# E3SM-Project/PAM

Hardware: AMD Instinct MI355X
Metric: cell-updates/sec (AWFL dycore step) (higher is better)
Workload: dtype f64; 1 GPU; AWFL supercell idealized, nens=1024/GPU, 32x32x60 L60, NT=1, fp64; scaling=weak, nens_total=1024, nens_per_gpu=1024, nx=32, ny=32, nz=60, num_tracers=1, parallelism=nens-shard x1, ranks_seen=1, limiter_input=0, fct_rows_flagged_last_stage=0, fct_rows=983040, lanes=member+xsweep

## Files before the change

### pam_amd/csrc/awfl_device.h

```cpp
#pragma once
#include <math.h>
#include <stdint.h>
#include <string.h>
#include <type_traits>
#include "awfl_constants.h"

#if defined(__HIPCC__)
#define PAMA_D __device__ __forceinline__
#else
#define PAMA_D inline
#endif

namespace pama {

constexpr int HS = 3;
constexpr int MAXT = 50;
constexpr int FLUX_THREADS = 256;
constexpr int FLUX_WAVES = FLUX_THREADS / 64;
#ifndef PAMA_FLUX_NF
#define PAMA_FLUX_NF 2
#endif
constexpr int FLUX_NF = PAMA_FLUX_NF;
constexpr int FLUX_MAX_SPAN = 64;
constexpr int VZ_STRIDE = 31;
// ... 1448 lines not shown
    for (int n = 0; n < NF; n++) T.nq[n] = uni(q[n] + on)[eu];
    T.ruf = uni(ruf_line + (long long)(c == nx ? 0 : c) * P.sx)[eu];
    const int cc = c > c0 ? c - 1 : c0;
    const long long o = pbase + (long long)cc * P.sx, ix = fbase + (long long)cc * P.sx;
    T.rho_in = 0.0; T.rho_0 = 0.0; T.rho_new = 1.0;
    if (PHASE == 2) {
      T.rho_in = uni(pr + o)[eu];
      T.rho_0 = (STAGE > 1) ? uni(r0 + o)[eu] : 0.0;
      T.rho_new = uni(rn + o)[eu];
    }
#pragma unroll
    for (int n = 0; n < NF; n++) {
      T.yl[n] = have_y ? uni(fyt[n] + ix)[eu] : 0.0;
      T.yh[n] = have_y ? uni(fyt[n] + ix + jp1)[eu] : 0.0;
      T.zl[n] = uni(fzt[n] + ix)[eu];
      T.zh[n] = uni(fzt[n] + ix + P.sz)[eu];
      T.sd[n] = (PHASE == 1) ? uni(seed + (long long)tt[n] * P.ncell + ix)[eu] : 0.0;
      T.q_0[n] = (PHASE == 2 && STAGE > 1) ? uni(q0p[n] + o)[eu] : 0.0;
      T.m_jm1[n] = T.m_jp1[n] = T.m_km1[n] = T.m_kp1[n] = T.m_new[n] = 1.0;
      if (PHASE == 2) {
        T.m_new[n] = uni(mline[n] + (long long)(c == nx ? 0 : c) * P.sx)[eu];
        if (have_y) { T.m_jm1[n] = uni(mline[n] + (long long)cc * P.sx + jm1)[eu]; T.m_jp1[n] = uni(mline[n] + (long long)cc * P.sx + jp1)[eu]; }
        if (zlo) T.m_km1[n] = uni(mline[n] + (long long)cc * P.sx - P.sz)[eu];
        if (zhi) T.m_kp1[n] = uni(mline[n] + (long long)cc * P.sx + P.sz)[eu];
      }
    }
  };
  Trip Tn;
  if (AHEAD) load_trip(c0, Tn);
#pragma clang loop unroll(disable)
  for (int c = c0; c <= c1; c++) {
    Trip T;
    if (AHEAD) {
      T = Tn;
      if (c < c1) load_trip(c + 1, Tn);
    } else {
      load_trip(c, T);
    }
    double L[NF], R[NF];
    double ruf = T.ruf;
    if (have_close && c == c1) ruf = ruf_close;
    const int cc = c > c0 ? c - 1 : c0;
    const long long ix = fbase + (long long)cc * P.sx;
    const double rho_in = T.rho_in, rho_0 = T.rho_0, rho_new = T.rho_new;
    const double (&nq)[NF] = T.nq, (&yl)[NF] = T.yl, (&yh)[NF] = T.yh, (&zl)[NF] = T.zl, (&zh)[NF] = T.zh, (&sd)[NF] = T.sd, (&q_0)[NF] = T.q_0;
    const double (&m_new)[NF] = T.m_new, (&m_jm1)[NF] = T.m_jm1, (&m_jp1)[NF] = T.m_jp1, (&m_km1)[NF] = T.m_km1, (&m_kp1)[NF] = T.m_kp1;
#pragma unroll
    for (int n = 0; n < NF; n++) weno5_const(w[n], wc, L[n], R[n]);
    const bool up = ruf > 0.0;
    const double rrho = (PHASE == 2) ? fast_rcp(rho_new) : 0.0;
#pragma unroll
    for (int n = 0; n < NF; n++) {
      const double F = mul_rn(ruf, up ? prevR[n] : L[n]);
      if (c > c0) {
        if (PHASE == 1) {
          own_multiplier_cell<true>(P, tt[n], mult, rows, k, j, cc, e, eu, ix, F_prev[n], F, yl[n], yh[n], zl[n], zh[n], sd[n], dzk, rdzk, dt_stage);
        } else {
          const double f_x = limited_flux(F_prev[n], mA[n], mB[n], cc == 0);
          const double f_xp1 = limited_flux(F, mB[n], m_new[n], cc == nx - 1);
          double f_y = 0.0, f_yp1 = 0.0;
          if (have_y) {
            f_y = limited_flux(yl[n], m_jm1[n], mB[n], j == 0);
            f_yp1 = limited_flux(yh[n], mB[n], m_jp1[n], j == P.ny - 1);
          }
          const double f_z = limited_flux(zl[n], m_km1[n], mB[n], false);
          const double f_zp1 = limited_flux(zh[n], mB[n], m_kp1[n], false);
          double v, new_seed;
          tracer_new_value<STAGE>(P, tt[n], f_x, f_xp1, f_y, f_yp1, f_z, f_zp1, w[n][1], q_0[n], rho_in, rho_0, rdzk, dt_dyn, v, new_seed);
          uniw(seed + (long long)tt[n] * P.ncell + ix)[eu] = new_seed;
          store_adv_u(P, prim_out, P_TR0 + tt[n], k, cu0 + (long long)cc * P.sx, eu, v * rrho, v * rrho);
        }
      }
      F_prev[n] = F;
      prevR[n] = R[n];
      mA[n] = mB[n];
      mB[n] = m_new[n];
#pragma unroll
      for (int s = 0; s < 4; s++) w[n][s] = w[n][s + 1];
      w[n][4] = nq[n];
    }
  }
}

template <int STAGE, bool FOLD = false>
PAMA_D void flux_x_update_body(const Params &P, const double *__restrict__ prim_in, const double *__restrict__ prim0,
                               double *__restrict__ prim_out, double *__restrict__ fx, const double *__restrict__ fy,
                               const double *__restrict__ fz, double *__restrict__ seed, double *__restrict__ mult,
                               const FctRows &rows, int line, int e, int c0, int span, double dt_dyn, double dt_stage,
                               bool tracers_inline) {
  const unsigned eu = member_offset(e);
  const WenoConsts wc = weno_consts();
  const int nx = P.nx;
  const int c1 = (c0 + span < nx) ? c0 + span : nx;
  const int k = uni_int(line / P.ny), j = line - k * P.ny;
  const long long cu0 = (long long)j * P.sy;
  const long long pbase = (long long)(k + HS) * P.sz + cu0;
  const long long fbase = (long long)k * P.sz + cu0;
  const long long jp1 = (j == P.ny - 1) ? -(long long)(P.ny - 1) * P.sy : P.sy;
  const long long ke = (long long)k * P.nens + e;
  const double dzk = P.dz[ke];
  const double rdzk = fast_rcp(dzk);
  const double gcoef = gravity_coef(P, ke);
  const bool have_y = !P.sim2d;
  double ruf_close = 0.0;
  double *ruf_line = fx + fbase;
  auto cell_off = [&](int c) -> long long { return pbase + (long long)(c < 0 ? c + nx : (c >= nx ? c - nx : c)) * P.sx; };

  {
    constexpr int NQ = 4;
    const double *pr = prim_in + (long long)P_RHO * P.prim_fs;
    const double *pp = prim_in + (long long)P_PRES * P.prim_fs;
    const double *r0 = prim0 + (long long)P_RHO * P.prim_fs;
    double *out_rho = prim_out + (long long)P_RHO * P.prim_fs, *out_rt = prim_out + (long long)P_PRES * P.prim_fs;
    double wm[5], wp[5], wq[NQ][5], wt[5];
    const int tr = P.idWV;
    const double *pt = prim_in + (long long)(P_TR0 + tr) * P.prim_fs;
    double *flt = fx + (long long)(5 + tr) * P.ncell + fbase;
    const bool more_tracers = P.nt > 1;
    auto load_cell = [&](long long o, double &m, double &p, double (&qv)[NQ]) {
#pragma unroll
      for (int n = 0; n < NQ; n++) qv[n] = uni(prim_in + (long long)(P_U + n) * P.prim_fs + o)[eu];
      m = mul_rn(uni(pr + o)[eu], qv[0]);
      p = uni(pp + o)[eu];
    };
#pragma unroll
    for (int s = 0; s < 5; s++) {
      double qv[NQ];
      load_cell(cell_off(c0 - 3 + s), wm[s], wp[s], qv);
#pragma unroll
      for (int n = 0; n < NQ; n++) wq[n][s] = qv[n];
      wt[s] = uni(pt + cell_off(c0 - 3 + s))[eu];
    }
    double prevR_m, prevR_p, prevR_q[NQ], prevR_t;
    {
      double L;
      weno5_const(wm, wc, L, prevR_m);
      weno5_const(wp, wc, L, prevR_p);
      weno5_const(wt, wc, L, prevR_t);
#pragma unroll
      for (int n = 0; n < NQ; n++) {
        if (n == 1 && !have_y) { prevR_q[n] = 0.0; continue; }
        weno5_const(wq[n], wc, L, prevR_q[n]);
      }
      double nm, np_, nq[NQ];
      load_cell(cell_off(c0 + 2), nm, np_, nq);
      const double nt0 = uni(pt + cell_off(c0 + 2))[eu];
#pragma unroll
      for (int s = 0; s < 4; s++) {
        wm[s] = wm[s + 1]; wp[s] = wp[s + 1]; wt[s] = wt[s + 1];
#pragma unroll
        for (int n = 0; n < NQ; n++) wq[n][s] = wq[n][s + 1];
      }
      wm[4] = nm; wp[4] = np_; wt[4] = nt0;
#pragma unroll
      for (int n = 0; n < NQ; n++) wq[n][4] = nq[n];
    }
    double F_prev[1 + NQ], Ft_prev = 0.0;
#pragma unroll
    for (int l = 0; l <= NQ; l++) F_prev[l] = 0.0;
    struct CellIn { double rho_in, rho_0, q0[NQ], y0l, y0h, z0l, z0h, dy[1 + NQ], dz[1 + NQ], tyl, tyh, tzl, tzh, tseed, tq0; };
    const double *fyt = fy + (long long)(5 + tr) * P.ncell, *fzt = fz + (long long)(5 + tr) * P.fz_fs;
    const double *pt0 = prim0 + (long long)(P_TR0 + tr) * P.prim_fs;
    const double *sdt = seed + (long long)tr * P.ncell;
    auto load_in = [&](int cc, CellIn &ci) {
      const long long o = pbase + (long long)cc * P.sx, ix = fbase + (long long)cc * P.sx;
      ci.rho_in = uni(pr + o)[eu];
      ci.rho_0 = (STAGE > 1) ? uni(r0 + o)[eu] : 0.0;
#pragma unroll
      for (int n = 0; n < NQ; n++) ci.q0[n] = (STAGE > 1) ? uni(prim0 + (long long)(P_U + n) * P.prim_fs + o)[eu] : 0.0;
      ci.y0l = have_y ? uni(fy + ix)[eu] : 0.0;
      ci.y0h = have_y ? uni(fy + ix + jp1)[eu] : 0.0;
      ci.z0l = uni(fz + ix)[eu];
      ci.z0h = uni(fz + ix + P.sz)[eu];
#pragma unroll
      for (int l = 1; l <= NQ; l++) {
        ci.dy[l] = (have_y && !FOLD) ? uni(fy + (long long)l * P.ncell + ix)[eu] : 0.0;
        ci.dz[l] = (l == 2 && !have_y) ? 0.0 : uni(fz + (long long)l * P.fz_fs + ix)[eu];
      }
      ci.tyl = have_y ? uni(fyt + ix)[eu] : 0.0;
      ci.tyh = have_y ? uni(fyt + ix + jp1)[eu] : 0.0;
      ci.tzl = uni(fzt + ix)[eu];
      ci.tzh = uni(fzt + ix + P.sz)[eu];
      ci.tseed = uni(sdt + ix)[eu];
      ci.tq0 = (STAGE > 1) ? uni(pt0 + o)[eu] : 0.0;
    };
    auto finish = [&](int cc, const CellIn &ci, const double (&Flo)[1 + NQ], const double (&Fhi)[1 + NQ], double m_in_u,
                      double v_in, double w_in, double th_in, double Ft_lo, double Ft_hi, double qt_in) {
      const long long o = pbase + (long long)cc * P.sx;
      const double q0 = rk_combine<STAGE>(ci.rho_0, ci.rho_in, dt_dyn,
                                          flux_divergence(P, Flo[0], Fhi[0], ci.y0l, ci.y0h, ci.z0l, ci.z0h, rdzk));
      const double rrho = fast_rcp(q0);
      uniw(out_rho + o)[eu] = q0;
      const double q_in[NQ] = {0.0, v_in, w_in, th_in};
#pragma unroll
      for (int n = 0; n < NQ; n++) {
        const int l = 1 + n;
        double tend = FOLD ? flux_divergence_g(P, Flo[l], Fhi[l], ci.dz[l]) : flux_divergence_d(P, Flo[l], Fhi[l], ci.dy[l], ci.dz[l], rdzk);
        if (l == 3) tend = add_gravity(P, tend, ci.rho_in, gcoef);
        if (l == 2 && P.sim2d) tend = 0.0;
        const double m_in = (n == 0) ? m_in_u : mul_rn(q_in[n], ci.rho_in);
        const double m_0 = (STAGE > 1) ? mul_rn(ci.q0[n], ci.rho_0) : 0.0;
        const double v = rk_combine<STAGE>(m_0, m_in, dt_dyn, tend);
        store_adv_u(P, prim_out, P_U + n, k, cu0 + (long long)cc * P.sx, eu, v * rrho, (l == 3) ? 0.0 : v * rrho);
        if (l == 4) uniw(out_rt + o)[eu] = v;
      }
      finish_tracer_cell<STAGE>(P, tr, prim_out, seed, mult, rows, k, j, cc, e, eu, cu0 + (long long)cc * P.sx, fbase + (long long)cc * P.sx,
                                Ft_lo, Ft_hi, ci.tyl, ci.tyh, ci.tzl, ci.tzh, ci.tseed, qt_in, ci.tq0, ci.rho_in, ci.rho_0, rrho, dzk,
                                rdzk, dt_dyn, dt_stage);
    };
#pragma clang loop unroll(disable)
    for (int c = c0; c <= c1; c++) {
      double nm, np_, nq[NQ];
      load_cell(cell_off(c + 3), nm, np_, nq);
      const double nt0 = uni(pt + cell_off(c + 3))[eu];
      CellIn ci;
      load_in(c > c0 ? c - 1 : c0, ci);
      double Lm, Rm, Lp, Rp, Lq[NQ], Rq[NQ];
      weno5_const(wm, wc, Lm, Rm);
      weno5_const(wp, wc, Lp, Rp);
#pragma unroll
      for (int n = 0; n < NQ; n++) {
        if (n == 1 && !have_y) { Lq[n] = Rq[n] = 0.0; continue; }
        weno5_const(wq[n], wc, Lq[n], Rq[n]);
      }
      double Lt, Rt;
      weno5_const(wt, wc, Lt, Rt);
      double ruf, ppf, F[1 + NQ];
      acoustic_face(prevR_m, Lm, prevR_p, Lp, false, ruf, ppf);
      const bool up = ruf > 0.0;
      const double Ft = mul_rn(ruf, up ? prevR_t : Lt);
      if (c < c1) {
        if (more_tracers) uniw(ruf_line + (long long)c * P.sx)[eu] = ruf;
        uniw(flt + (long long)c * P.sx)[eu] = Ft;
      }
      ruf_close = ruf;
      F[0] = ruf;
      F[1] = fma(ruf, up ? prevR_q[0] : Lq[0], ppf);
#pragma unroll
      for (int n = 1; n < NQ; n++) F[1 + n] = mul_rn(ruf, up ? prevR_q[n] : Lq[n]);
      if (c > c0) finish(c - 1, ci, F_prev, F, wm[1], wq[1][1], wq[2][1], wq[3][1], Ft_prev, Ft, wt[1]);
#pragma unroll
      for (int l = 0; l <= NQ; l++) F_prev[l] = F[l];
      Ft_prev = Ft;
      prevR_m = Rm; prevR_p = Rp; prevR_t = Rt;
#pragma unroll
      for (int n = 0; n < NQ; n++) prevR_q[n] = Rq[n];
#pragma unroll
      for (int s = 0; s < 4; s++) {
        wm[s] = wm[s + 1]; wp[s] = wp[s + 1]; wt[s] = wt[s + 1];
#pragma unroll
        for (int n = 0; n < NQ; n++) wq[n][s] = wq[n][s + 1];
      }
      wm[4] = nm; wp[4] = np_; wt[4] = nt0;
#pragma unroll
      for (int n = 0; n < NQ; n++) wq[n][4] = nq[n];
    }
  }

  if (tracers_inline) {
    for (int i = 0; i < P.nt - 1; i += FLUX_NF) {
      const int fa[2] = {4 + further_tracer(P, i), 4 + further_tracer(P, i + 1)};
      if (i + 1 < P.nt - 1) x_tracer_sweep<2, STAGE, 1>(P, prim_in, prim0, prim_out, fx, fy, fz, seed, mult, rows, line, e, c0, span, fa, dt_dyn, dt_stage, true, ruf_close);
      else x_tracer_sweep<1, STAGE, 1>(P, prim_in, prim0, prim_out, fx, fy, fz, seed, mult, rows, line, e, c0, span, fa, dt_dyn, dt_stage, true, ruf_close);
    }
  }
}

struct XTileGeom {
  int W;
  int nmb;
  int tc;
  int halo;
  int ntl;
  int lpb;
};
PAMA_HD int xtile_rows(const XTileGeom &G) { return G.tc + 2 * G.halo; }
PAMA_HD int xtile_threads(const XTileGeom &G) { return G.W * xtile_rows(G) * G.lpb; }
PAMA_HD XTileGeom xtile_geometry(const Params &P, int w_req, int tc_req, int lpb_req, int ncu = 0) {
  XTileGeom G;
  G.W = (P.nens <= 64) ? P.nens : 64;
  if (P.nens < 64 && (long long)P.nx * P.nens > 512) {
    const int nmb = (int)(((long long)P.nx * P.nens + 511) / 512), w = (P.nens + nmb - 1) / nmb;
    if (w >= 16 && P.nx * w <= 1024) G.W = w;
    else if ((long long)P.nx * P.nens > 1024) {
      const int nmb2 = (int)(((long long)P.nx * P.nens + 1023) / 1024), w2 = (P.nens + nmb2 - 1) / nmb2;
      if (w2 >= 16 && P.nx * w2 <= 1024) G.W = w2;
    }
  }
  if (w_req > 0) G.W = w_req < P.nens ? w_req : P.nens;
  if (G.W > 1024 / 3) G.W = 64;
  G.nmb = (P.nens + G.W - 1) / G.W;
  const int max_threads = 1024;
  if (tc_req <= 0 && P.nx * G.W <= max_threads) {
    G.halo = 0; G.tc = P.nx; G.ntl = 1;
    const int row = P.nx * G.W, most = max_threads / row;
    auto used = [&](int l) { return (double)(l * row) / (double)(((l * row + 63) / 64) * 64); };
    double best = 0.0;
    for (int l = 1; l <= most; l++) best = used(l) > best ? used(l) : best;
    G.lpb = most;
    for (int l = 1; l <= most; l++)
      if (used(l) >= best - 0.03 && (l * row >= 192 || l == most)) { G.lpb = l; break; }
    if (ncu > 0) {
      const long long nlines = (long long)P.nz * P.ny;
      long long best_cost = -1;
      int best_dist = 0;
      for (int l = 1; l <= most; l++) {
        if (used(l) < best - 0.03) continue;
        const int T = ((l * row + 63) / 64) * 64;
        const long long nwg = (long long)G.nmb * ((nlines + l - 1) / l);
        const long long cost = ((nwg + ncu - 1) / ncu) * T;
        const int dist = T > 256 ? T - 256 : 256 - T;
        if (best_cost < 0 || cost < best_cost || (cost == best_cost && dist < best_dist)) { best_cost = cost; best_dist = dist; G.lpb = l; }
      }
    }
    if (lpb_req > 0) G.lpb = lpb_req < most ? lpb_req : most;
    if (G.lpb < 1) G.lpb = 1;
  } else {
    G.halo = 1; G.lpb = 1;
    int tc = tc_req > 0 ? tc_req : 14;
    if (tc > P.nx) tc = P.nx;
    while (tc > 1 && (tc + 2) * G.W > max_threads) tc--;
    G.ntl = (P.nx + tc - 1) / tc;
    G.tc = tc_req > 0 ? tc : (P.nx + G.ntl - 1) / G.ntl;
  }
  return G;
}
PAMA_HD bool xtile_supported(const Params &P) { return P.prim_fs < (1ll << 28) && P.fz_fs < (1ll << 28) && (long long)P.nz * P.ny < (1ll << 30); }

struct XLane {
  int k, j, i, e;
  bool poly, face, upd;
  int slot, slot_l, slot_r;
  unsigned po, io, ke;
  int s5[5];
  int nstage;
  unsigned stage_po[3];
  int stage_el[3];
};
// ... 732 lines not shown
```

### pam_amd/csrc/awfl_kernels.hip

```cpp
#include <hip/hip_runtime.h>

#include <cmath>
#include <cstdio>
#include <cstring>
#include <atomic>
#include <map>
#include <mutex>
#include <string>
#include <vector>

#include "../../include/pam_amd_awfl.h"
#include "awfl_device.h"
#include "awfl_vertical.h"

using namespace pama;

struct EnsRange { int e0, ne; };
__device__ __forceinline__ long long to_global(long long t, int nens, EnsRange R) {
  const long long r = t / R.ne;
  return r * nens + R.e0 + (t - r * R.ne);
}

__device__ __forceinline__ bool flat_cell(const Params &P, int nlev, CellId &c) {
  const unsigned t = blockIdx.x * blockDim.x + threadIdx.x;
// ... 82 lines not shown
  double *buf;
  const double *vz;
  long long nens;
  int eb, emax;
  int tid, lane, last;
  double r[(VZ_STRIDE * 64 + 64 * ZPE_WAVES - 1) / (64 * ZPE_WAVES)];
  static constexpr int NR = (VZ_STRIDE * 64 + 64 * ZPE_WAVES - 1) / (64 * ZPE_WAVES);
  __device__ __forceinline__ double rdz(const Params &P, int k, int e) const { return P.rdz[(long long)k * P.nens + e]; }
  __device__ __forceinline__ void load(int level) {
    const double *src = vz + (long long)level * VZ_STRIDE * nens;
#pragma unroll
    for (int i = 0; i < NR; i++) {
      const int idx = tid + i * 64 * ZPE_WAVES;
      const int m = idx >> 6, l = idx & 63, em = (eb + l < emax) ? eb + l : emax;
      r[i] = (idx < VZ_STRIDE * 64) ? src[(long long)m * nens + em] : 0.0;
    }
  }
  __device__ __forceinline__ void store(int level) {
    double *dst = buf + (level & 1) * (VZ_STRIDE * 64);
#pragma unroll
    for (int i = 0; i < NR; i++) {
      const int idx = tid + i * 64 * ZPE_WAVES;
      if (idx < VZ_STRIDE * 64) dst[idx] = r[i];
    }
  }
  __device__ __forceinline__ void pass_begin(int first, int last_) {
    last = last_;
    load(first);
    store(first);
    __syncthreads();
  }
  __device__ __forceinline__ void trip_begin(int level) { if (level < last) load(level + 1); }
  __device__ __forceinline__ void trip_end(int level) {
    if (level < last) store(level + 1);
    __syncthreads();
  }
  __device__ __forceinline__ void weno(const double u[5], int level, const WenoConsts &wc, double &L, double &R) const {
    weno5_table(u, buf + (level & 1) * (VZ_STRIDE * 64) + lane, 64, wc, L, R);
  }
};
template <bool DIFF, bool FOLD>
__global__ void __launch_bounds__(64 * ZPE_WAVES, 2) awfl_fluxz_pe_kernel(Params P, EnsRange R, int spz, int nsz, int part, int npz,
                                                                              const double *__restrict__ prim, const double *__restrict__ fy,
                                                                              double *__restrict__ fz) {
  __shared__ double ztab[2 * VZ_STRIDE * 64];
  const int lane = threadIdx.x & 63;
  const int wave = __builtin_amdgcn_readfirstlane((int)(threadIdx.x >> 6));
  const int ncol = P.ny * P.nx, ncg = (ncol + ZPE_WAVES - 1) / ZPE_WAVES;
  const int per_blk = ncg * nsz * (part == 1 ? npz : 1);
  const int b = (int)blockIdx.x;
  const int blk = uni_int(b / per_blk), r1 = b - blk * per_blk;
  const int r2 = uni_int(r1 / ncg), cg = r1 - r2 * ncg;
  const int pp = uni_int(r2 / nsz), sp = r2 - pp * nsz;
  const int psel = (part == 1) ? 1 + pp : part;
  int line = cg * ZPE_WAVES + wave;
  if (line > ncol - 1) line = ncol - 1;
  const int emax = R.e0 + R.ne - 1;
  int e = R.e0 + blk * 64 + lane;
  if (e > emax) e = emax;
  ZTabLds zt;
  zt.buf = ztab; zt.vz = P.vz; zt.nens = P.nens; zt.eb = R.e0 + blk * 64; zt.emax = emax;
  zt.tid = (int)threadIdx.x; zt.lane = lane; zt.last = 0;
  flux_line_body_zt<2, DIFF, ZTabLds, FOLD>(P, prim, fz, member_lane<2>(P, line, e), sp * spz, spz, psel, zt, fy);
}

__global__ void __launch_bounds__(256) awfl_fct_kernel(Params P, EnsRange R, const double *__restrict__ fx,
                                                       const double *__restrict__ fy, const double *__restrict__ fz,
                                                       const double *__restrict__ seed, double *__restrict__ mult,
                                                       FctRows rows, double dt, int t0) {
  fct_rows_resolve(rows);
  CellId c;
  if (grid_cell(P, R, c)) fct_mult_body(P, fx, fy, fz, seed, mult, rows, dt, c, t0);
}
template <int STAGE>
__global__ void __launch_bounds__(256) awfl_update_kernel(Params P, EnsRange R, const double *prim_in,
                                                          const double *prim0, double *prim_out,
                                                          const double *__restrict__ fx, const double *__restrict__ fy,
                                                          const double *__restrict__ fz, const double *__restrict__ mult,
                                                          FctRows rows, double *__restrict__ seed, double dt_dyn) {
  fct_rows_resolve(rows);
  CellId c;
  if (grid_cell(P, R, c)) update_body<STAGE>(P, prim_in, prim0, prim_out, fx, fy, fz, mult, rows, seed, dt_dyn, c);
}
template <int STAGE, bool FOLD>
__global__ void __launch_bounds__(FLUX_THREADS, 2) awfl_xupd_kernel(Params P, EnsRange R, const double *__restrict__ prim_in,
                                                                     const double *__restrict__ prim0,
                                                                     double *__restrict__ prim_out, double *__restrict__ fx,
                                                                     const double *__restrict__ fy,
                                                                     const double *__restrict__ fz, double *__restrict__ seed,
                                                                     double *__restrict__ mult, FctRows rows, double dt_dyn,
                                                                     double dt_stage, int tracers_inline, int span, int nspan) {
  fct_rows_resolve(rows);
  const int u = __builtin_amdgcn_readfirstlane((int)(blockIdx.x * FLUX_WAVES + (threadIdx.x >> 6)));
  const SweepUnits U = sweep_units(P.nz, P.ny, R.ne, nspan, 1);
  const SweepUnits::Unit w = U.decode(u, false);
  const int sp = U.span(w);
  const SweepUnits::Lane m = U.place(w.grp);
  const int el = m.blk * 64 + (int)(threadIdx.x & 63);
  if (U.holds(m, el))
    flux_x_update_body<STAGE, FOLD>(P, prim_in, prim0, prim_out, fx, fy, fz, seed, mult, rows, m.line, R.e0 + el, sp * span, span,
                                    dt_dyn, dt_stage, tracers_inline != 0);
}
template <int STAGE, int PHASE, int G, bool AHEAD = false>
__device__ __forceinline__ void xtr_block(const Params &P, EnsRange R, const double *__restrict__ prim_in,
                                          const double *__restrict__ prim0, double *__restrict__ prim_out,
                                          const double *__restrict__ fx, const double *__restrict__ fy,
                                          const double *__restrict__ fz, double *__restrict__ seed,
                                          double *__restrict__ mult, const FctRows &rows, double dt_dyn,
                                          double dt_stage, int ngroups, int span, int nspan, int block) {
  static_assert(G == 1 || G == 2 || G == 4, "one, two or four tracers per wavefront");
  static_assert(!AHEAD || G == 2, "the one-trip-ahead form exists for pairs only");
  const int u = __builtin_amdgcn_readfirstlane((int)(block * FLUX_WAVES + (threadIdx.x >> 6)));
  const SweepUnits U = sweep_units(P.nz, P.ny, R.ne, nspan, ngroups);
  const SweepUnits::Unit w = U.decode(u);
  const int sp = U.span(w);
  const SweepUnits::Lane m = U.place(w.grp);
  const int el = m.blk * 64 + (int)(threadIdx.x & 63);
  if (!U.holds(m, el)) return;
  if constexpr (G == 2) {
    const int fa[2] = {4 + further_tracer(P, 2 * w.sel), 4 + further_tracer(P, 2 * w.sel + 1)};
    if (2 * w.sel + 1 < P.nt - 1)
      x_tracer_sweep<2, STAGE, PHASE, AHEAD>(P, prim_in, prim0, prim_out, fx, fy, fz, seed, mult, rows, m.line, R.e0 + el, sp * span, span, fa, dt_dyn, dt_stage, false, 0.0);
    else
      x_tracer_sweep<1, STAGE, PHASE, AHEAD>(P, prim_in, prim0, prim_out, fx, fy, fz, seed, mult, rows, m.line, R.e0 + el, sp * span, span, fa, dt_dyn, dt_stage, false, 0.0);
  } else {
    const int first = G * w.sel, left = P.nt - 1 - first;
    const int fa[4] = {4 + further_tracer(P, first), 4 + further_tracer(P, first + 1), 4 + further_tracer(P, first + 2), 4 + further_tracer(P, first + 3)};
    if (G == 4 && left >= 4)
      x_tracer_sweep<4, STAGE, PHASE, AHEAD>(P, prim_in, prim0, prim_out, fx, fy, fz, seed, mult, rows, m.line, R.e0 + el, sp * span, span, fa, dt_dyn, dt_stage, false, 0.0);
    else if (G == 4 && left == 3)
      x_tracer_sweep<3, STAGE, PHASE, AHEAD>(P, prim_in, prim0, prim_out, fx, fy, fz, seed, mult, rows, m.line, R.e0 + el, sp * span, span, fa, dt_dyn, dt_stage, false, 0.0);
    else if (G == 4 && left == 2)
      x_tracer_sweep<2, STAGE, PHASE, AHEAD>(P, prim_in, prim0, prim_out, fx, fy, fz, seed, mult, rows, m.line, R.e0 + el, sp * span, span, fa, dt_dyn, dt_stage, false, 0.0);
    else
      x_tracer_sweep<1, STAGE, PHASE, AHEAD>(P, prim_in, prim0, prim_out, fx, fy, fz, seed, mult, rows, m.line, R.e0 + el, sp * span, span, fa, dt_dyn, dt_stage, false, 0.0);
  }
}
template <int STAGE, int PHASE, int G, bool AHEAD = false>
__global__ void __launch_bounds__(FLUX_THREADS) awfl_xtr_kernel(Params P, EnsRange R, const double *__restrict__ prim_in,
                                                               const double *__restrict__ prim0, double *__restrict__ prim_out,
                                                               const double *__restrict__ fx, const double *__restrict__ fy,
                                                               const double *__restrict__ fz, double *__restrict__ seed,
                                                               double *__restrict__ mult, FctRows rows, double dt_dyn,
                                                               double dt_stage, int ngroups, int span, int nspan) {
  fct_rows_resolve(rows);
  xtr_block<STAGE, PHASE, G, AHEAD>(P, R, prim_in, prim0, prim_out, fx, fy, fz, seed, mult, rows, dt_dyn, dt_stage, ngroups, span, nspan,
                                    (int)blockIdx.x);
}
constexpr int TAIL_LEVELS = 6;
__device__ __forceinline__ void stage_pow_tab(Params &P, PowTab *sh_tab) {
  const double *src = reinterpret_cast<const double *>(P.pw);
  double *dst = reinterpret_cast<double *>(sh_tab);
  for (int i = threadIdx.x; i < (int)(sizeof(PowTab) / sizeof(double)); i += blockDim.x) dst[i] = src[i];
  __syncthreads();
  P.pw = sh_tab;
}
__device__ __forceinline__ void ptail_block(const Params &P, EnsRange R, double *__restrict__ prim_out, unsigned bx, int by, int bz) {
  const unsigned t = bx * blockDim.x + threadIdx.x;
  if (t >= (unsigned)P.nx * (unsigned)R.ne) return;
  CellId c;
  const unsigned i = t / (unsigned)R.ne;
  c.j = by; c.i = (int)i; c.e = R.e0 + (int)(t - i * (unsigned)R.ne);
#pragma unroll
  for (int kk = 0; kk < TAIL_LEVELS; kk++) {
    c.k = bz * TAIL_LEVELS + kk;
    if (c.k >= P.nz) return;
    c.idx = (((long long)c.k * P.ny + c.j) * P.nx + c.i) * P.nens + c.e;
    pressure_tail_body(P, prim_out, c);
  }
}
__global__ void __launch_bounds__(256) awfl_ptail_kernel(Params P, EnsRange R, double *__restrict__ prim_out) {
  __shared__ PowTab sh_tab;
  stage_pow_tab(P, &sh_tab);
  if (!P.flat_cells) { ptail_block(P, R, prim_out, blockIdx.x, (int)blockIdx.y, (int)blockIdx.z); return; }
  CellId c;
  const int ngrp = (P.nz + TAIL_LEVELS - 1) / TAIL_LEVELS;
  if (!flat_cell(P, ngrp, c)) return;
  const int kg = c.k;
#pragma unroll
  for (int kk = 0; kk < TAIL_LEVELS; kk++) {
    c.k = kg * TAIL_LEVELS + kk;
    if (c.k >= P.nz) return;
    c.idx = (((long long)c.k * P.ny + c.j) * P.nx + c.i) * P.nens + c.e;
    pressure_tail_body(P, prim_out, c);
// ... 995 lines not shown

inline int further_tracer_pairs(const Params &P) { return (P.nt - 1 + 1) / 2; }

inline size_t xtile_lds_bytes(const XTileGeom &G, int fields) { return (size_t)fields * (xtile_threads(G) + xtile_stage_elems(G)) * sizeof(double); }
inline bool xtile_lds_fits(const XTileGeom &G) { return xtile_lds_bytes(G, XT_NS) <= 160 * 1024; }

struct XupdResult {
  int rc; bool tail_fused;
  XupdResult(int rc_, bool tail_fused_ = false) : rc(rc_), tail_fused(tail_fused_) {}
};

int launch_xupd_tiles(pam_amd_awfl *h, const StageArgs &a, EnsRange r, hipStream_t s) {
  const Params &P = h->P;
  if (r.e0 != 0 || r.ne != P.nens) return fail(PAM_AMD_EINVAL, "x-tile launch: the tile kernels take the whole ensemble in one range");
  const XTileGeom &G = h->use.xg;
  const dim3 block((unsigned)G.W, (unsigned)xtile_rows(G), (unsigned)G.lpb);
  const dim3 grid((unsigned)(G.ntl * G.nmb), (unsigned)((P.nz * P.ny + G.lpb - 1) / G.lpb), 1);
  if (grid.y > 65535u) return fail(PAM_AMD_EINVAL, "x-tile launch: more than 65535 groups of x lines");
  const bool lds = !h->use.xshuf;
  if (lds && !xtile_lds_fits(G)) return fail(PAM_AMD_EINVAL, "x-tile launch: the staged tile does not fit the 160 KB of LDS");
  const size_t lds_state = lds ? xtile_lds_bytes(G, XT_NS) : 0, lds_pair = lds ? xtile_lds_bytes(G, 2) : 0;
  const bool wave_is_row = (G.W == 64 && P.nens % 64 == 0);
  const int npairs = further_tracer_pairs(P), pressure = h->use.tile_pressure ? 1 : 0;
  int rc;
  {
    const int sparts = (pressure && h->use.tile_state_parts) ? 1 : 0;
    const int tr_mode = pressure ? (((h->use.tile_tracers_parallel || sparts) && npairs > 0 && npairs < 65535) ? 2 : 1) : 0;
    const dim3 sgrid(grid.x, grid.y, (unsigned)((sparts ? 3 : 1) + (tr_mode == 2 ? npairs : 0)));
    const auto kernel = lds ? by_stage(a.st, [](auto S) { return awfl_xupd_tile_kernel<S(), false>; })
                            : by_stage(a.st, [](auto S) { return awfl_xupd_tile_kernel<S(), true>; });
    if ((rc = launch(h, "xupd", kernel, sgrid, block, lds_state, s, P, G, a.in, a.base, a.out, h->flux_x, h->flux_y, h->flux_z, h->seed, h->mult,
                     fct_rows(h, r, wave_is_row), a.dt_dyn, a.dt_stage, pressure, tr_mode, sparts)))
      return rc;
  }
  if (npairs > 65535) return fail(PAM_AMD_EINVAL, "x-tile launch: too many tracer pairs");
  if (npairs == 0) return PAM_AMD_OK;
  if (!pressure) {
    const auto kernel = lds ? by_stage(a.st, [](auto S) { return awfl_xtr_tile_kernel<S(), 1, false>; })
                            : by_stage(a.st, [](auto S) { return awfl_xtr_tile_kernel<S(), 1, true>; });
    if ((rc = launch(h, "xtr1", kernel, dim3(grid.x, grid.y, (unsigned)npairs), block, lds_pair, s, P, G, a.in, a.base, a.out, h->flux_x, h->flux_y,
                     h->flux_z, h->seed, h->mult, fct_rows(h, r, wave_is_row), a.dt_dyn, a.dt_stage, 0)))
      return rc;
  }
  const auto kernel = lds ? by_stage(a.st, [](auto S) { return awfl_xtr_tile_kernel<S(), 2, false>; })
                            : by_stage(a.st, [](auto S) { return awfl_xtr_tile_kernel<S(), 2, true>; });
  return launch(h, "xtr2", kernel, dim3(grid.x, grid.y, (unsigned)(npairs + pressure)), block, lds_pair, s, P, G, a.in, a.base, a.out, h->flux_x,
                h->flux_y, h->flux_z, h->seed, h->mult, fct_rows(h, r, wave_is_row), a.dt_dyn, a.dt_stage, pressure);
}

struct TracerSweepShape { int per, span; SweepUnits U; };
TracerSweepShape tracer_sweep_shape(const pam_amd_awfl *h, EnsRange r, int per) {
  const Params &P = h->P;
  TracerSweepShape T;
  T.per = per;
  const int ngroups = per == 4 ? (P.nt - 1 + 3) / 4 : (per == 1 ? P.nt - 1 : further_tracer_pairs(P));
  int nspan;
  choose_span(h, P.nx, (long long)P.nz * P.ny * ngroups, P.nens, P.seg, h->span_override, T.span, nspan, 2);
  T.U = sweep_units(P.nz, P.ny, r.ne, nspan, ngroups);
  return T;
}

auto xtr_kernel(int st, int phase, int per, bool ahead) {
  const auto phase1 = by_stage(st, [&](auto S) {
    return per == 4 ? awfl_xtr_kernel<S(), 1, 4> : per == 1 ? awfl_xtr_kernel<S(), 1, 1> : awfl_xtr_kernel<S(), 1, 2>;
  });
  const auto phase2 = by_stage(st, [&](auto S) {
    return per == 4 ? awfl_xtr_kernel<S(), 2, 4> : per == 1 ? awfl_xtr_kernel<S(), 2, 1> : ahead ? awfl_xtr_kernel<S(), 2, 2, true> : awfl_xtr_kernel<S(), 2, 2>;
  });
  return phase == 1 ? phase1 : phase2;
}

XupdResult launch_xupd_sweeps(pam_amd_awfl *h, const StageArgs &a, EnsRange r, hipStream_t s, bool allow_tail_fusion) {
  const Params &P = h->P;
  int span, nspan, rc;
  choose_span(h, P.nx, (long long)P.nz * P.ny, P.nens, P.seg, h->span_override, span, nspan);
  const SweepUnits U = sweep_units(P.nz, P.ny, r.ne, nspan, 1);
  const int npairs = further_tracer_pairs(P);
  const bool split = npairs > 0 && sweep_units(P.nz, P.ny, P.nens, nspan, 1).count() < h->split_below;
  if (!sweep_units(P.nz, P.ny, r.ne, nspan, npairs > 0 ? npairs : 1).fits()) return fail(PAM_AMD_EINVAL, "x-sweep launch: more than 2^30 wavefronts");
  if (r.e0 % 64) return fail(PAM_AMD_EINVAL, "x-sweep launch: member ranges of the fused stage start at multiples of 64 (a wavefront is one row of FCT flags)");
  const dim3 block(FLUX_THREADS);
  {
    const auto kernel = by_stage(a.st, [&](auto S) { return P.yz_fold ? awfl_xupd_kernel<S(), true> : awfl_xupd_kernel<S(), false>; });
    if ((rc = launch(h, "xupd", kernel, dim3((unsigned)U.workgroups(FLUX_WAVES)), block, 0, s, P, r, a.in, a.base, a.out, h->flux_x, h->flux_y, h->flux_z,
                     h->seed, h->mult, fct_rows(h, r, true), a.dt_dyn, a.dt_stage, split ? 0 : 1, span, nspan)))
      return rc;
  }
  if (npairs == 0) return PAM_AMD_OK;
  const int per1 = h->tracers_per_wave ? h->tracers_per_wave : 1;
  const int per2 = h->tracers_per_wave ? h->tracers_per_wave : (P.nt - 1 == 3 ? 1 : 2);
  auto launch_tracer_sweep = [&](int phase, const TracerSweepShape &T) {
    return launch(h, phase == 1 ? "xtr1" : "xtr2", xtr_kernel(a.st, phase, T.per, h->tracer_prefetch), dim3((unsigned)T.U.workgroups(FLUX_WAVES)),
                  block, 0, s, P, r, a.in, a.base, a.out, h->flux_x, h->flux_y, h->flux_z, h->seed, h->mult, fct_rows(h, r, true), a.dt_dyn,
                  a.dt_stage, T.U.nsel, T.span, T.U.nspan);
  };
  if (split) {
    if ((rc = launch_tracer_sweep(1, tracer_sweep_shape(h, r, per1)))) return rc;
  }
  const TracerSweepShape T = tracer_sweep_shape(h, r, per2);
  if (allow_tail_fusion && (h->want.tail_fuse == 2 || T.U.count() < 6144)) {
    const long long nb_xtr = T.U.workgroups(FLUX_WAVES);
    const dim3 pg = cell_grid(P, r, (P.nz + TAIL_LEVELS - 1) / TAIL_LEVELS);
    const long long nb_pt = (long long)pg.x * pg.y * pg.z;
    const long long nb_fix = sweep_units(P.nz, P.ny, r.ne, 1, 1).workgroups(4);
    if (nb_xtr + nb_pt + nb_fix > 0x7fffffffll) return fail(PAM_AMD_EINVAL, "tail launch: more than 2^31 workgroups");
    const auto kernel = by_stage(a.st, [&](auto S) { return T.per == 1 ? awfl_xtr2_tail_kernel<S(), true> : awfl_xtr2_tail_kernel<S(), false>; });
    rc = launch(h, "xtr2", kernel, dim3((unsigned)(nb_xtr + nb_pt + nb_fix)), block, 0, s, P, r, a.in, a.base, a.out, h->flux_x, h->flux_y, h->flux_z,
                h->seed, h->mult, fct_rows(h, r, true), fct_rows(h, r, false), a.dt_dyn, a.dt_stage, T.U.nsel, T.span, T.U.nspan, (int)nb_xtr,
                (int)nb_pt, (int)pg.x);
    return XupdResult(rc, true);
  }
  return launch_tracer_sweep(2, T);
}

XupdResult launch_xupd(pam_amd_awfl *h, const StageArgs &a, EnsRange r, hipStream_t s, bool allow_tail_fusion) {
  if (h->use.xtile) return launch_xupd_tiles(h, a, r, s);
  return launch_xupd_sweeps(h, a, r, s, allow_tail_fusion);
}

int launch_tail(pam_amd_awfl *h, const StageArgs &a, EnsRange r, hipStream_t s) {
  const Params &P = h->P;
  const bool in_tile = h->use.xtile && h->use.tile_pressure;
  if (!in_tile)
    if (int rc = launch(h, "ptail", awfl_ptail_kernel, cell_grid(P, r, (P.nz + TAIL_LEVELS - 1) / TAIL_LEVELS), dim3(256), 0, s, P, r, a.out)) return rc;
  if (in_tile && P.nt > 1) return PAM_AMD_OK;
  if (P.flat_cells)
    return launch(h, "trfix", by_stage(a.st, [](auto S) { return awfl_trfix_flat_kernel<S()>; }), cell_grid(P, r), dim3(256), 0, s, P, a.in, a.base,
                  a.out, h->flux_x, h->flux_y, h->flux_z, h->mult, fct_rows(h, r, false), h->seed, a.dt_dyn);
  const SweepUnits U = sweep_units(P.nz, P.ny, r.ne, 1, 1);
  if (!U.fits()) return fail(PAM_AMD_EINVAL, "fix-up launch: more than 2^30 wavefronts");
  return launch(h, "trfix", by_stage(a.st, [](auto S) { return awfl_trfix_kernel<S()>; }), dim3((unsigned)U.workgroups(4)), dim3(256), 0, s, P, r, a.in,
                a.base, a.out, h->flux_x, h->flux_y, h->flux_z, h->mult, fct_rows(h, r, false), h->seed, a.dt_dyn);
}

int launch_mass(pam_amd_awfl *h, int slot, EnsRange r, hipStream_t s) {
  const Params &P = h->P;
  return launch(h, nullptr, awfl_mass_kernel, dim3((unsigned)((r.ne + 63) / 64), (unsigned)(P.nt + 2)), dim3(256), 0, s, P, r, h->prim0, h->seed,
                h->mass_dev + (size_t)slot * (P.nt + 2) * P.nens);
}
int evaluate_mass(pam_amd_awfl *h) {
  const Params &P = h->P;
  const size_t n = (size_t)(P.nt + 2) * P.nens;
  std::vector<double> m(2 * n);
  HIP_TRY(hipStreamSynchronize(h->stream));
  HIP_TRY(hipMemcpy(m.data(), h->mass_dev, 2 * n * sizeof(double), hipMemcpyDeviceToHost));
  h->mass_violations = 0; h->mass_max_rel = 0.0; h->mass_worst_var = h->mass_worst_member = -1;
  h->mass_report.clear();
  for (int ivar = 0; ivar < P.nt + 2; ivar++)
    for (int e = 0; e < P.nens; e++) {
      const double a = m[(size_t)ivar * P.nens + e], b = m[n + (size_t)ivar * P.nens + e];
      const double ad = std::fabs(b - a), rd = ad / (std::fabs(a) + 1.e-20);
      const bool bad = !(rd <= 1.e-10) && !(ad <= 1.e-10);
      if (rd > h->mass_max_rel || (rd != rd && h->mass_worst_var < 0)) { h->mass_max_rel = rd; h->mass_worst_var = ivar; h->mass_worst_member = e; }
      if (!bad) continue;
      h->mass_violations++;
      if (h->mass_violations <= 32) {
        char line[256];
        std::snprintf(line, sizeof(line), "WARNING: conservation violated variable,ensemble,rel_diff,mass_diff,init,final: %d , %d , %.6e , %.6e , %.6e , %.6e\n",
                      ivar, e, rd, b - a, a, b);
        h->mass_report += line;
      }
    }
  return PAM_AMD_OK;
}

int launch_cfl(pam_amd_awfl *h, const pam_amd_awfl_fields_t *f, double cfl, bool lean) {
  if (!f || !f->tracers) return fail(PAM_AMD_EINVAL, "fields: null pointer");
// ... 1123 lines not shown
```

Before: 2.680 billion cell-updates/s.

## Sweep periodic x-lines in one pass, stashing wrap-around face state in LDS

When one wavefront covers the whole periodic x-line, the sweep now starts at cell 0 rather than c0-1. The left-edge reconstruction and the first face flux are stashed in LDS, then reused to close the wrap-around cells nx-1 and 0 at the end. This drops the duplicated halo WENO reconstructions and face evaluation at the line start. The cost is 13 doubles of LDS per lane (about 26 KB per workgroup) and an epilogue with two extra finish calls, which could reduce occupancy.

```diff
diff --git a/pam_amd/csrc/awfl_device.h b/pam_amd/csrc/awfl_device.h
--- a/pam_amd/csrc/awfl_device.h
+++ b/pam_amd/csrc/awfl_device.h
@@ -1554,16 +1554,26 @@
   }
 }
 
-template <int STAGE, bool FOLD = false>
+constexpr int XSWEEP_STASH = 13;
+constexpr int XSWEEP_ONE_PASS_MIN_NX = 5;
+PAMA_HD bool xsweep_one_pass(int nx, int c0, int span) { return c0 == 0 && span >= nx && nx >= XSWEEP_ONE_PASS_MIN_NX; }
+struct LocalStash {
+  double v[XSWEEP_STASH];
+  PAMA_HD void put(int slot, double x) { v[slot] = x; }
+  PAMA_HD double get(int slot) const { return v[slot]; }
+};
+template <int STAGE, bool FOLD = false, class Stash = LocalStash>
 PAMA_D void flux_x_update_body(const Params &P, const double *__restrict__ prim_in, const double *__restrict__ prim0,
                                double *__restrict__ prim_out, double *__restrict__ fx, const double *__restrict__ fy,
                                const double *__restrict__ fz, double *__restrict__ seed, double *__restrict__ mult,
                                const FctRows &rows, int line, int e, int c0, int span, double dt_dyn, double dt_stage,
-                               bool tracers_inline) {
+                               bool tracers_inline, Stash stash = Stash()) {
   const unsigned eu = member_offset(e);
   const WenoConsts wc = weno_consts();
   const int nx = P.nx;
   const int c1 = (c0 + span < nx) ? c0 + span : nx;
+  const bool one_pass = xsweep_one_pass(nx, c0, span);
+  const int cs = one_pass ? 0 : c0 - 1;
   const int k = uni_int(line / P.ny), j = line - k * P.ny;
   const long long cu0 = (long long)j * P.sy;
   const long long pbase = (long long)(k + HS) * P.sz + cu0;
@@ -1598,35 +1608,12 @@
 #pragma unroll
     for (int s = 0; s < 5; s++) {
       double qv[NQ];
-      load_cell(cell_off(c0 - 3 + s), wm[s], wp[s], qv);
+      load_cell(cell_off(cs - 2 + s), wm[s], wp[s], qv);
 #pragma unroll
       for (int n = 0; n < NQ; n++) wq[n][s] = qv[n];
-      wt[s] = uni(pt + cell_off(c0 - 3 + s))[eu];
+      wt[s] = uni(pt + cell_off(cs - 2 + s))[eu];
     }
     double prevR_m, prevR_p, prevR_q[NQ], prevR_t;
-    {
-      double L;
-      weno5_const(wm, wc, L, prevR_m);
-      weno5_const(wp, wc, L, prevR_p);
-      weno5_const(wt, wc, L, prevR_t);
-#pragma unroll
-      for (int n = 0; n < NQ; n++) {
-        if (n == 1 && !have_y) { prevR_q[n] = 0.0; continue; }
-        weno5_const(wq[n], wc, L, prevR_q[n]);
-      }
-      double nm, np_, nq[NQ];
-      load_cell(cell_off(c0 + 2), nm, np_, nq);
-      const double nt0 = uni(pt + cell_off(c0 + 2))[eu];
-#pragma unroll
-      for (int s = 0; s < 4; s++) {
-        wm[s] = wm[s + 1]; wp[s] = wp[s + 1]; wt[s] = wt[s + 1];
-#pragma unroll
-        for (int n = 0; n < NQ; n++) wq[n][s] = wq[n][s + 1];
-      }
-      wm[4] = nm; wp[4] = np_; wt[4] = nt0;
-#pragma unroll
-      for (int n = 0; n < NQ; n++) wq[n][4] = nq[n];
-    }
     double F_prev[1 + NQ], Ft_prev = 0.0;
 #pragma unroll
     for (int l = 0; l <= NQ; l++) F_prev[l] = 0.0;
@@ -1680,13 +1667,41 @@
                                 Ft_lo, Ft_hi, ci.tyl, ci.tyh, ci.tzl, ci.tzh, ci.tseed, qt_in, ci.tq0, ci.rho_in, ci.rho_0, rrho, dzk,
                                 rdzk, dt_dyn, dt_stage);
     };
-#pragma clang loop unroll(disable)
-    for (int c = c0; c <= c1; c++) {
+    auto face = [&](int cf, bool own, double Lm, double Lp, const double (&Lq)[NQ], double Lt, double (&F)[1 + NQ], double &Ft)
+                    __attribute__((always_inline)) {
+      double ruf, ppf;
+      acoustic_face(prevR_m, Lm, prevR_p, Lp, false, ruf, ppf);
+      const bool up = ruf > 0.0;
+      Ft = mul_rn(ruf, up ? prevR_t : Lt);
+      if (own) {
+        if (more_tracers) uniw(ruf_line + (long long)cf * P.sx)[eu] = ruf;
+        uniw(flt + (long long)cf * P.sx)[eu] = Ft;
+      }
+      ruf_close = ruf;
+      F[0] = ruf;
+      F[1] = fma(ruf, up ? prevR_q[0] : Lq[0], ppf);
+#pragma unroll
+      for (int n = 1; n < NQ; n++) F[1 + n] = mul_rn(ruf, up ? prevR_q[n] : Lq[n]);
+    };
+    auto shift = [&](double nm, double np_, const double (&nq)[NQ], double nt0) __attribute__((always_inline)) {
+#pragma unroll
+      for (int s = 0; s < 4; s++) {
+        wm[s] = wm[s + 1]; wp[s] = wp[s + 1]; wt[s] = wt[s + 1];
+#pragma unroll
+        for (int n = 0; n < NQ; n++) wq[n][s] = wq[n][s + 1];
+      }
+      wm[4] = nm; wp[4] = np_; wt[4] = nt0;
+#pragma unroll
+      for (int n = 0; n < NQ; n++) wq[n][4] = nq[n];
+    };
+    constexpr int EDGES = 0, FACE = 1, CLOSE = 2;
+    auto trip = [&](int c, auto what_tag) __attribute__((always_inline)) {
+      constexpr int WHAT = decltype(what_tag)::value;
       double nm, np_, nq[NQ];
       load_cell(cell_off(c + 3), nm, np_, nq);
       const double nt0 = uni(pt + cell_off(c + 3))[eu];
       CellIn ci;
-      load_in(c > c0 ? c - 1 : c0, ci);
+      if (WHAT == CLOSE) load_in(c - 1, ci);
       double Lm, Rm, Lp, Rp, Lq[NQ], Rq[NQ];
       weno5_const(wm, wc, Lm, Rm);
       weno5_const(wp, wc, Lp, Rp);
@@ -1697,35 +1712,52 @@
       }
       double Lt, Rt;
       weno5_const(wt, wc, Lt, Rt);
-      double ruf, ppf, F[1 + NQ];
-      acoustic_face(prevR_m, Lm, prevR_p, Lp, false, ruf, ppf);
-      const bool up = ruf > 0.0;
-      const double Ft = mul_rn(ruf, up ? prevR_t : Lt);
-      if (c < c1) {
-        if (more_tracers) uniw(ruf_line + (long long)c * P.sx)[eu] = ruf;
-        uniw(flt + (long long)c * P.sx)[eu] = Ft;
+      if (WHAT == EDGES) {
+        if (one_pass) {
+          stash.put(0, Lm); stash.put(1, Lp); stash.put(2, Lt);
+#pragma unroll
+          for (int n = 0; n < NQ; n++) stash.put(3 + n, Lq[n]);
+        }
+      } else {
+        double F[1 + NQ], Ft;
+        face(c, c < c1, Lm, Lp, Lq, Lt, F, Ft);
+        if (WHAT == CLOSE) finish(c - 1, ci, F_prev, F, wm[1], wq[1][1], wq[2][1], wq[3][1], Ft_prev, Ft, wt[1]);
+#pragma unroll
+        for (int l = 0; l <= NQ; l++) F_prev[l] = F[l];
+        Ft_prev = Ft;
       }
-      ruf_close = ruf;
-      F[0] = ruf;
-      F[1] = fma(ruf, up ? prevR_q[0] : Lq[0], ppf);
-#pragma unroll
-      for (int n = 1; n < NQ; n++) F[1 + n] = mul_rn(ruf, up ? prevR_q[n] : Lq[n]);
-      if (c > c0) finish(c - 1, ci, F_prev, F, wm[1], wq[1][1], wq[2][1], wq[3][1], Ft_prev, Ft, wt[1]);
-#pragma unroll
-      for (int l = 0; l <= NQ; l++) F_prev[l] = F[l];
-      Ft_prev = Ft;
       prevR_m = Rm; prevR_p = Rp; prevR_t = Rt;
 #pragma unroll
       for (int n = 0; n < NQ; n++) prevR_q[n] = Rq[n];
-#pragma unroll
-      for (int s = 0; s < 4; s++) {
-        wm[s] = wm[s + 1]; wp[s] = wp[s + 1]; wt[s] = wt[s + 1];
-#pragma unroll
-        for (int n = 0; n < NQ; n++) wq[n][s] = wq[n][s + 1];
+      shift(nm, np_, nq, nt0);
+    };
+    trip(cs, std::integral_constant<int, EDGES>());
+    trip(cs + 1, std::integral_constant<int, FACE>());
+    if (one_pass) {
+#pragma unroll
+      for (int l = 0; l <= NQ; l++) stash.put(7 + l, F_prev[l]);
+      stash.put(12, Ft_prev);
+    }
+    const int c_last = one_pass ? nx - 1 : c1;
+#pragma clang loop unroll(disable)
+    for (int c = cs + 2; c <= c_last; c++) trip(c, std::integral_constant<int, CLOSE>());
+    if (one_pass) {
+      double Lq[NQ], F[1 + NQ], Ft;
+#pragma unroll
+      for (int n = 0; n < NQ; n++) Lq[n] = stash.get(3 + n);
+      face(0, true, stash.get(0), stash.get(1), Lq, stash.get(2), F, Ft);
+#pragma clang loop unroll(disable)
+      for (int t = 0; t < 2; t++) {
+        const int cc = t ? 0 : nx - 1;
+        CellIn ci;
+        load_in(cc, ci);
+        finish(cc, ci, F_prev, F, wm[1], wq[1][1], wq[2][1], wq[3][1], Ft_prev, Ft, wt[1]);
+#pragma unroll
+        for (int l = 0; l <= NQ; l++) { F_prev[l] = F[l]; F[l] = stash.get(7 + l); }
+        Ft_prev = Ft; Ft = stash.get(12);
+        const double none[NQ] = {0.0, 0.0, 0.0, 0.0};
+        shift(0.0, 0.0, none, 0.0);
       }
-      wm[4] = nm; wp[4] = np_; wt[4] = nt0;
-#pragma unroll
-      for (int n = 0; n < NQ; n++) wq[n][4] = nq[n];
     }
   }
 
diff --git a/pam_amd/csrc/awfl_kernels.hip b/pam_amd/csrc/awfl_kernels.hip
--- a/pam_amd/csrc/awfl_kernels.hip
+++ b/pam_amd/csrc/awfl_kernels.hip
@@ -188,6 +188,14 @@
   CellId c;
   if (grid_cell(P, R, c)) update_body<STAGE>(P, prim_in, prim0, prim_out, fx, fy, fz, mult, rows, seed, dt_dyn, c);
 }
+struct XupdLdsStash {
+  double *p;
+  __device__ __forceinline__ void put(int slot, double x) { p[slot * 64] = x; }
+  __device__ __forceinline__ double get(int slot) const { return p[slot * 64]; }
+};
+static size_t xupd_stash_bytes(int nx, int span) {
+  return pama::xsweep_one_pass(nx, 0, span) ? (size_t)FLUX_WAVES * pama::XSWEEP_STASH * 64 * sizeof(double) : 0;
+}
 template <int STAGE, bool FOLD>
 __global__ void __launch_bounds__(FLUX_THREADS, 2) awfl_xupd_kernel(Params P, EnsRange R, const double *__restrict__ prim_in,
                                                                      const double *__restrict__ prim0,
@@ -203,9 +211,11 @@
   const int sp = U.span(w);
   const SweepUnits::Lane m = U.place(w.grp);
   const int el = m.blk * 64 + (int)(threadIdx.x & 63);
+  extern __shared__ double xupd_lds[];
+  const XupdLdsStash stash{xupd_lds + (threadIdx.x >> 6) * (XSWEEP_STASH * 64) + (threadIdx.x & 63)};
   if (U.holds(m, el))
     flux_x_update_body<STAGE, FOLD>(P, prim_in, prim0, prim_out, fx, fy, fz, seed, mult, rows, m.line, R.e0 + el, sp * span, span,
-                                    dt_dyn, dt_stage, tracers_inline != 0);
+                                    dt_dyn, dt_stage, tracers_inline != 0, stash);
 }
 template <int STAGE, int PHASE, int G, bool AHEAD = false>
 __device__ __forceinline__ void xtr_block(const Params &P, EnsRange R, const double *__restrict__ prim_in,
@@ -1367,7 +1377,7 @@
   const dim3 block(FLUX_THREADS);
   {
     const auto kernel = by_stage(a.st, [&](auto S) { return P.yz_fold ? awfl_xupd_kernel<S(), true> : awfl_xupd_kernel<S(), false>; });
-    if ((rc = launch(h, "xupd", kernel, dim3((unsigned)U.workgroups(FLUX_WAVES)), block, 0, s, P, r, a.in, a.base, a.out, h->flux_x, h->flux_y, h->flux_z,
+    if ((rc = launch(h, "xupd", kernel, dim3((unsigned)U.workgroups(FLUX_WAVES)), block, xupd_stash_bytes(P.nx, span), s, P, r, a.in, a.base, a.out, h->flux_x, h->flux_y, h->flux_z,
                      h->seed, h->mult, fct_rows(h, r, true), a.dt_dyn, a.dt_stage, split ? 0 : 1, span, nspan)))
       return rc;
   }
```

New measurement: 2.707 billion cell-updates/s, median of 6. +1.0%, better.
